# utra-robosoccer/Bez_IsaacGym

Measured on AMD Instinct MI355X. Metric: env-steps/s at num_envs=4096 (random-action rollout, bez_kick), higher is better.
Workload: dtype f32

## Files before the change

### bez_isaacgym_amd/csrc/bez_policy.hip

```cpp
#include <hip/hip_fp16.h>
#include <hip/hip_runtime.h>
#include <stdint.h>
#include <cstdlib>
#include <cstring>

#include <type_traits>

#include "../../include/bez_sim.h"
#include "bez_dr_noise.h"
#include "bez_dr_step.h"
#include "bez_ppo_loss.h"

namespace {

using half8 = __attribute__((ext_vector_type(8))) _Float16;
using f32x16 = __attribute__((ext_vector_type(16))) float;
using f32x2 = __attribute__((ext_vector_type(2))) float;
using half2v = __attribute__((ext_vector_type(2))) _Float16;
using half4v = __attribute__((ext_vector_type(4))) _Float16;

constexpr int PF_ROWS = 64;
constexpr int PF_MAXW = 416;
constexpr int PF_LD = PF_MAXW + 8;
constexpr int PF_MAXL = 6;
constexpr int PF_WAVES = 8;

struct PolicyArgs {
  const float* obs; int64_t n; int d_in;
  const double* mean; const double* var; float eps;
  int nhid;
  const _Float16* w[PF_MAXL]; const _Float16* b[PF_MAXL]; int width[PF_MAXL];
  const _Float16* w_mu; const _Float16* b_mu; int num_actions;
  const _Float16* w_val; const _Float16* b_val;
  float* mu; float* value;
  const float* logstd; const float* noise; const float* dones; const double* vmean; const double* vvar; float veps;
  float* mb_obs; float* mb_dones; float* mb_mu; float* mb_val; float* act; float* act_env; float* neglogp; float* sigma;
  BezPpoRolloutPost post;
  BezPpoActionNoise an;
  int dr_on; bez::dr::DrArgs dr;
  int64_t ld_obs, ld_act, ld_one;
  _Float16* x0_out; _Float16* act_out[PF_MAXL];
  int packed;
#ifdef BEZ_PF_STAMPS
  unsigned long long* stamps;
#endif
};
#ifdef BEZ_PF_STAMPS
#define PF_STAMP(k) do { if (a.stamps && blockIdx.x == 0 && threadIdx.x == 0) a.stamps[k] = __builtin_amdgcn_s_memtime(); } while (0)
__device__ unsigned long long* g_pf_wave_stamps = nullptr;
#define PF_WSTAMP(tag, wave, ph) do { if (g_pf_wave_stamps && blockIdx.x == 0 && (threadIdx.x & 63) == 0) g_pf_wave_stamps[(tag) * 64 + (wave) * 4 + (ph)] = __builtin_amdgcn_s_memtime(); } while (0)
#else
#define PF_STAMP(k) do { } while (0)
#define PF_WSTAMP(tag, wave, ph) do { } while (0)
#endif

template <int LD>
__device__ __forceinline__ void store_tile(const _Float16 (*src)[LD], _Float16* dst, int64_t row0, int nrow, int cols, int tid, int nw = PF_WAVES) {
  const int lane = tid & 63, wave = tid >> 6;
  if ((cols & 3) == 0) {
    const int c4 = cols >> 2;
    for (int rr = wave; rr < nrow; rr += nw) {
      _Float16* drow = dst + (row0 + rr) * cols;
      for (int c = lane; c < c4; c += 64) *reinterpret_cast<uint2*>(drow + 4 * c) = *reinterpret_cast<const uint2*>(&src[rr][4 * c]);
    }
  } else {
    const int c2 = cols >> 1;
    for (int rr = wave; rr < nrow; rr += nw) {
      _Float16* drow = dst + (row0 + rr) * cols;
      for (int c = lane; c < c2; c += 64) *reinterpret_cast<uint32_t*>(drow + 2 * c) = *reinterpret_cast<const uint32_t*>(&src[rr][2 * c]);
    }
  }
}

struct __attribute__((packed, aligned(4))) H8 { _Float16 v[8]; };

__device__ __forceinline__ half8 load_w8(const _Float16* row, int k0, int cols) {
  half8 f;
  if (k0 + 8 <= cols && (cols & 1) == 0) {
    const H8 t = *reinterpret_cast<const H8*>(row + k0);
#pragma unroll
    for (int j = 0; j < 8; ++j) f[j] = t.v[j];
  } else {
#pragma unroll
    for (int j = 0; j < 8; ++j) f[j] = (k0 + j < cols) ? row[k0 + j] : (_Float16)0.f;
  }
  return f;
}

template <int LD>
__device__ __forceinline__ void gemm_col_block(const _Float16 (*src)[LD], const _Float16* wrow, bool live, int in, int r, int h, f32x16& acc0, f32x16& acc1) {
  const int full = ((in & 1) == 0) ? (in >> 4) : 0;
  const int ksteps = (in + 15) >> 4;
  int ks = 0;
  auto group = [&](auto G) {
    constexpr int g = decltype(G)::value;
    half8 bf[g];
#pragma unroll
    for (int u = 0; u < g; ++u) {
      if (live) {
        const H8 t = *reinterpret_cast<const H8*>(wrow + (ks + u) * 16 + 8 * h);
#pragma unroll
        for (int j = 0; j < 8; ++j) bf[u][j] = t.v[j];
      } else {
#pragma unroll
        for (int j = 0; j < 8; ++j) bf[u][j] = (_Float16)0.f;
      }
    }
#pragma unroll
    for (int u = 0; u < g; ++u) {
      const int k0 = (ks + u) * 16 + 8 * h;
      const half8 a0 = *reinterpret_cast<const half8*>(&src[r][k0]);
      const half8 a1 = *reinterpret_cast<const half8*>(&src[32 + r][k0]);
      acc0 = __builtin_amdgcn_mfma_f32_32x32x16_f16(a0, bf[u], acc0, 0, 0, 0);
      acc1 = __builtin_amdgcn_mfma_f32_32x32x16_f16(a1, bf[u], acc1, 0, 0, 0);
    }
    ks += g;
  };
  while (ks + 12 <= full) group(std::integral_constant<int, 12>{});
  while (ks + 4 <= full) group(std::integral_constant<int, 4>{});
  while (ks + 1 <= full) group(std::integral_constant<int, 1>{});
  for (; ks < ksteps; ++ks) {
    const int k0 = ks * 16 + 8 * h;
    const half8 bf = load_w8(wrow, k0, live ? in : 0);
    const half8 a0 = *reinterpret_cast<const half8*>(&src[r][k0]);
    const half8 a1 = *reinterpret_cast<const half8*>(&src[32 + r][k0]);
    acc0 = __builtin_amdgcn_mfma_f32_32x32x16_f16(a0, bf, acc0, 0, 0, 0);
    acc1 = __builtin_amdgcn_mfma_f32_32x32x16_f16(a1, bf, acc1, 0, 0, 0);
  }
}

struct alignas(4) BiasQuad { half2v lo, hi; };
struct Bias16 { BiasQuad q[4]; };
__device__ __forceinline__ Bias16 load_bias16(const _Float16* B, int cb, int out) {
  Bias16 b;
  const half2v z = half2v{(_Float16)0.f, (_Float16)0.f};
  if (!B) {
#pragma unroll
    for (int j = 0; j < 4; ++j) { b.q[j].lo = z; b.q[j].hi = z; }
  } else if (((out & 3) | (int)(reinterpret_cast<uintptr_t>(B) & 3)) == 0) {
#pragma unroll
    for (int j = 0; j < 4; ++j) {
      const int c = cb + 8 * j;
      b.q[j] = *reinterpret_cast<const BiasQuad*>(B + (c < out ? c : 0));
    }
  } else {
#pragma unroll
    for (int j = 0; j < 4; ++j) {
      const int c = cb + 8 * j;
      b.q[j].lo = half2v{B[c < out ? c : 0], B[c + 1 < out ? c + 1 : 0]};
      b.q[j].hi = half2v{B[c + 2 < out ? c + 2 : 0], B[c + 3 < out ? c + 3 : 0]};
    }
  }
  return b;
}
constexpr int PF_G = 4;
template <int LD, bool T, int NACC, int RP>
__device__ __forceinline__ void gemm_packed(const _Float16 (*src)[LD], const _Float16* wblk, int ksteps, int r, int h, int half, f32x16* acc,
                                            const Bias16* bias = nullptr) {
  const _Float16* p = wblk + (h * 32 + r) * 8;
  auto fetch = [&](half8* f, int g) {
#pragma unroll
    for (int u = 0; u < PF_G; ++u) {
      const int k = g * PF_G + u < ksteps ? g * PF_G + u : ksteps - 1;
      f[u] = *reinterpret_cast<const half8*>(p + (size_t)k * 512);
    }
    __builtin_amdgcn_sched_barrier(0);
  };
  auto mma = [&](const half8& w, int ks) {
    const int k0 = ks * 16 + 8 * h;
    if (NACC == 2) {
      const half8 a0 = *reinterpret_cast<const half8*>(&src[r][k0]);
      const half8 a1 = *reinterpret_cast<const half8*>(&src[32 + r][k0]);
      acc[0] = T ? __builtin_amdgcn_mfma_f32_32x32x16_f16(w, a0, acc[0], 0, 0, 0) : __builtin_amdgcn_mfma_f32_32x32x16_f16(a0, w, acc[0], 0, 0, 0);
      acc[NACC - 1] = T ? __builtin_amdgcn_mfma_f32_32x32x16_f16(w, a1, acc[NACC - 1], 0, 0, 0) : __builtin_amdgcn_mfma_f32_32x32x16_f16(a1, w, acc[NACC - 1], 0, 0, 0);
    } else {
      const half8 a0 = *reinterpret_cast<const half8*>(&src[32 * half + r][k0]);
      acc[0] = T ? __builtin_amdgcn_mfma_f32_32x32x16_f16(w, a0, acc[0], 0, 0, 0) : __builtin_amdgcn_mfma_f32_32x32x16_f16(a0, w, acc[0], 0, 0, 0);
    }
  };
  auto stage = [&](const half8* f, int ks, auto CNT) {
#pragma unroll
    for (int u = 0; u < decltype(CNT)::value; ++u) mma(f[u], ks + u);
    __builtin_amdgcn_sched_barrier(0);
  };
  using Full = std::integral_constant<int, PF_G>;
  const int npair = ksteps / (2 * PF_G);
  half8 fa[PF_G], fb[PF_G];
  __builtin_amdgcn_sched_barrier(0);
  fetch(fa, 0);
#pragma unroll
  for (int j = 0; j < 4; ++j) {
    f32x2 lo = {0.f, 0.f}, hi = {0.f, 0.f};
    if (T && bias) { lo = __builtin_convertvector(bias->q[j].lo, f32x2); hi = __builtin_convertvector(bias->q[j].hi, f32x2); }
#pragma unroll
    for (int c = 0; c < NACC; ++c) { acc[c][4 * j] = lo.x; acc[c][4 * j + 1] = lo.y; acc[c][4 * j + 2] = hi.x; acc[c][4 * j + 3] = hi.y; }
  }
  __builtin_amdgcn_sched_barrier(0);
  for (int i = 0; i < npair; ++i) {
    fetch(fb, 2 * i + 1);
    stage(fa, 2 * i * PF_G, Full{});
    fetch(fa, 2 * i + 2);
    stage(fb, (2 * i + 1) * PF_G, Full{});
  }
  if constexpr (RP > PF_G) fetch(fb, 2 * npair + 1);
  if constexpr (RP > 0) stage(fa, 2 * npair * PF_G, std::integral_constant<int, (RP < PF_G ? RP : PF_G)>{});
  if constexpr (RP > PF_G) stage(fb, (2 * npair + 1) * PF_G, std::integral_constant<int, RP - PF_G>{});
}
template <class F>
__device__ __forceinline__ void dispatch_ksteps(int ksteps, F&& run) {
  static_assert(PF_G == 4, "eight remainders");
  switch (ksteps & 7) {
    case 0: run(std::integral_constant<int, 0>{}); break;
    case 1: run(std::integral_constant<int, 1>{}); break;
    case 2: run(std::integral_constant<int, 2>{}); break;
    case 3: run(std::integral_constant<int, 3>{}); break;
    case 4: run(std::integral_constant<int, 4>{}); break;
    case 5: run(std::integral_constant<int, 5>{}); break;
    case 6: run(std::integral_constant<int, 6>{}); break;
    default: run(std::integral_constant<int, 7>{}); break;
  }
}
template <bool ELU, int LDD>
__device__ __forceinline__ void store_row_groups(const f32x16& acc, _Float16 (*dst)[LDD], int row, int cb, int npad) {
#pragma unroll
  for (int j = 0; j < 4; ++j) {
    const int c0 = cb + 8 * j;
    uint32_t o[2];
#pragma unroll
    for (int q = 0; q < 2; ++q) {
      const int i = 4 * j + 2 * q;
      const half2v hq = __builtin_convertvector(f32x2{acc[i], acc[i + 1]}, half2v);
      if (ELU) {
        const f32x2 e = f32x2{__builtin_amdgcn_exp2f(__builtin_fmaf((float)hq.x, 1.4426950408889634f, 0.f)),
                              __builtin_amdgcn_exp2f(__builtin_fmaf((float)hq.y, 1.4426950408889634f, 0.f))} - f32x2{1.f, 1.f};
        const half2v eh = __builtin_convertvector(e, half2v);
        const uint32_t hb = __builtin_bit_cast(uint32_t, hq), eb = __builtin_bit_cast(uint32_t, eh);
        uint32_t neg;
        asm("v_pk_ashrrev_i16 %0, %1, %2" : "=v"(neg) : "v"(0x000f000fu), "v"(hb));
        o[q] = (eb & neg) | (hb & ~neg);
      } else {
        o[q] = __builtin_bit_cast(uint32_t, hq);
      }
    }
    if (LDD >= PF_LD || c0 < npad) *reinterpret_cast<uint2*>(&dst[row][c0]) = make_uint2(o[0], o[1]);
  }
}

template <bool ELU, bool PK, bool ONEHALF = false, int LDS, int LDD>
__device__ __forceinline__ void layer(const _Float16 (*src)[LDS], _Float16 (*dst)[LDD], const _Float16* W, const _Float16* B, int in, int out, int wave,
                                      int lane, int tag = 0, int nw = PF_WAVES) {
  const int r = lane & 31, h = lane >> 5;
  const int nblk = (out + 31) >> 5, npad = (out + 15) & ~15;
  if constexpr (PK && ONEHALF) {
    const int ksteps = (in + 15) >> 4;
    dispatch_ksteps(ksteps, [&](auto RP) {
      for (int nb = wave; nb < nblk; nb += nw) {
        const int cb = nb * 32 + 4 * h;
        const Bias16 bias = load_bias16(B, cb, out);
        f32x16 acc;
        if (nb == wave) PF_WSTAMP(tag, wave, 0);
        gemm_packed<LDS, true, 1, decltype(RP)::value>(src, W + (size_t)nb * ksteps * 512, ksteps, r, h, 0, &acc, &bias);
        if (nb == wave) PF_WSTAMP(tag, wave, 1);
        store_row_groups<ELU>(acc, dst, r, cb, npad);
        if (nb == wave) PF_WSTAMP(tag, wave, 2);
      }
    });
    return;
  }
  if constexpr (PK) {
    const int ksteps = (in + 15) >> 4;
    if (nblk * 2 <= PF_WAVES) {
      if (wave < 2 * nblk) {
        const int nb = wave < nblk ? wave : wave - nblk, half = wave < nblk ? 0 : 1, cb = nb * 32 + 4 * h;
        dispatch_ksteps(ksteps, [&](auto RP) {
          const Bias16 bias = load_bias16(B, cb, out);
          f32x16 acc;
          PF_WSTAMP(tag, wave, 0);
          gemm_packed<LDS, true, 1, decltype(RP)::value>(src, W + (size_t)nb * ksteps * 512, ksteps, r, h, half, &acc, &bias);
          PF_WSTAMP(tag, wave, 1);
          store_row_groups<ELU>(acc, dst, 32 * half + r, cb, npad);
          PF_WSTAMP(tag, wave, 2);
        });
      }
      return;
    }
    dispatch_ksteps(ksteps, [&](auto RP) {
      for (int nb = wave; nb < nblk; nb += nw) {
        const int cb = nb * 32 + 4 * h;
        const Bias16 bias = load_bias16(B, cb, out);
        f32x16 acc[2];
        if (nb == wave) PF_WSTAMP(tag, wave, 0);
        gemm_packed<LDS, true, 2, decltype(RP)::value>(src, W + (size_t)nb * ksteps * 512, ksteps, r, h, 0, acc, &bias);
        if (nb == wave) PF_WSTAMP(tag, wave, 1);
        store_row_groups<ELU>(acc[0], dst, r, cb, npad);
        store_row_groups<ELU>(acc[1], dst, 32 + r, cb, npad);
        if (nb == wave) PF_WSTAMP(tag, wave, 2); else PF_WSTAMP(tag, wave, 3);
      }
    });
    return;
  }
  for (int nb = wave; nb < nblk; nb += nw) {
    const int n = nb * 32 + r;
    const _Float16* wrow = W + (size_t)(n < out ? n : 0) * in;
    const float bias = (B && n < out) ? (float)B[n] : 0.f;
    f32x16 acc0, acc1;
#pragma unroll
    for (int i = 0; i < 16; ++i) { acc0[i] = bias; acc1[i] = bias; }
    gemm_col_block(src, wrow, n < out, in, r, h, acc0, acc1);
#pragma unroll
    for (int i = 0; i < 16; ++i) {
      const int row = (i & 3) + 8 * (i >> 2) + 4 * h;
      float v0 = (float)(_Float16)acc0[i], v1 = (float)(_Float16)acc1[i];
      if (ELU) { v0 = v0 > 0.f ? v0 : __expf(v0) - 1.f; v1 = v1 > 0.f ? v1 : __expf(v1) - 1.f; }
      if (LDD >= PF_LD || n < npad) {
        dst[row][n] = (_Float16)v0;
        dst[32 + row][n] = (_Float16)v1;
      }
    }
  }
}

template <bool ROLL, bool PK, int LD>
__device__ __forceinline__ void heads(const PolicyArgs& a, const _Float16 (*src)[LD], int in, float* tile, int64_t row0, int nrow, int lane) {
  const int r = lane & 31, h = lane >> 5, A = a.num_actions;
  const _Float16* wrow = r < A ? a.w_mu + (size_t)r * in : a.w_val;
  const bool live = r <= A;
  f32x16 acc0, acc1;
#pragma unroll
  for (int i = 0; i < 16; ++i) { acc0[i] = 0.f; acc1[i] = 0.f; }
  static_assert(!PK, "the fragment-major instantiations use heads_half");
  gemm_col_block(src, wrow, live, in, r, h, acc0, acc1);
  const float bias = r < A ? (float)a.b_mu[r] : (r == A ? (float)a.b_val[0] : 0.f);
#pragma unroll
  for (int i = 0; i < 16; ++i) {
    const int row = (i & 3) + 8 * (i >> 2) + 4 * h;
    const float v0 = (float)(_Float16)(acc0[i] + bias), v1 = (float)(_Float16)(acc1[i] + bias);
    if (ROLL) {
      if (r <= A) { tile[row * 33 + r] = v0; tile[(32 + row) * 33 + r] = v1; }
    } else {
      if (row < nrow) { if (r < A) a.mu[(row0 + row) * A + r] = v0; else if (r == A) a.value[row0 + row] = v0; }
      if (32 + row < nrow) { if (r < A) a.mu[(row0 + 32 + row) * A + r] = v1; else if (r == A) a.value[row0 + 32 + row] = v1; }
    }
  }
}

__device__ __forceinline__ float head_bias(const PolicyArgs& a, int r) {
  return r < a.num_actions ? (float)a.b_mu[r] : (r == a.num_actions ? (float)a.b_val[0] : 0.f);
}
template <bool ROLL, int LD>
__device__ __forceinline__ void heads_half(const PolicyArgs& a, const _Float16 (*src)[LD], int in, float* tile, int64_t row0, int nrow, int lane, int half) {
  const int r = lane & 31, h = lane >> 5, A = a.num_actions, ksteps = (in + 15) >> 4;
  const float bias = head_bias(a, r);
  dispatch_ksteps(ksteps, [&](auto RP) {
    f32x16 acc;
    gemm_packed<LD, false, 1, decltype(RP)::value>(src, a.w_mu, ksteps, r, h, half, &acc);
#pragma unroll
    for (int i = 0; i < 16; ++i) {
      const int row = 32 * half + (i & 3) + 8 * (i >> 2) + 4 * h;
      const float v = (float)(_Float16)(acc[i] + bias);
      if (ROLL) {
        if (r <= A) tile[row * 33 + r] = v;
      } else if (row < nrow) {
        if (r < A) a.mu[(row0 + row) * A + r] = v; else if (r == A) a.value[row0 + row] = v;
      }
    }
  });
}

constexpr int PF_FWD_WAVES = 16;
template <int MODE, int LD0, int LD1, bool PK, int ROWS = PF_ROWS>
__global__ __launch_bounds__(MODE == 2 ? PF_WAVES * 64 : PF_FWD_WAVES * 64, (MODE != 2 || (LD0 + LD1) * PF_ROWS * 2 <= 80 * 1024) ? 4 : 2) void policy_forward_kernel(PolicyArgs a) {
  constexpr bool ROLL = MODE == 1, TRAIN = MODE == 2;
  static_assert(ROWS == PF_ROWS || (ROWS == 32 && PK && MODE != 2), "32-row tiles: fragment-major weights, forward-only / rollout kernels");
  constexpr bool ONEHALF = ROWS == 32;
  __shared__ __attribute__((aligned(16))) _Float16 t0[ROWS][LD0];
  __shared__ __attribute__((aligned(16))) _Float16 t1[ROWS][LD1];
  const int tid = threadIdx.x, lane = tid & 63, wave = tid >> 6;
  constexpr int nw = MODE == 2 ? PF_WAVES : PF_FWD_WAVES, nt = nw * 64;
  if (ROLL && a.dr_on && blockIdx.x == gridDim.x - 1) {
    int* scratch = reinterpret_cast<int*>(&t0[0][0]);
    constexpr int cap = (int)(sizeof(t0) / sizeof(int)) - 1;
    bez::dr::dr_step(a.dr, scratch + 1, cap, scratch);
    return;
  }
  const int64_t row0 = (int64_t)blockIdx.x * ROWS;
  const int nrow = (int)((a.n - row0) < (int64_t)ROWS ? (a.n - row0) : (int64_t)ROWS);
  PF_STAMP(0);
  __shared__ float nzs[ROLL ? ROWS * 32 : 1];
  if (ROLL && a.an.snap_dev) {
    const bez::DrSnap sn = *static_cast<const bez::DrSnap*>(a.an.snap_dev);
    const unsigned long long frame = (unsigned long long)sn.frame_hi << 32 | sn.frame_lo;
    const int nel = nrow * a.num_actions;
    for (int q = tid; 4 * q < nel; q += nt) {
      float z4[4];
      bez::dr_noise_quad(a.an.seed, a.an.env_id_offset, frame, 1, ((row0 * a.num_actions) >> 2) + q, z4);
#pragma unroll
      for (int c = 0; c < 4; ++c) nzs[4 * q + c] = fmaf(z4[c], sn.sd, sn.mean);
    }
  }
  const int kpad0 = (a.d_in + 15) & ~15;
  for (int k = lane; k < kpad0; k += 64) {
    const bool kin = k < a.d_in;
    float mk = 0.f, sk = 1.f;
    if (a.mean && kin) { mk = (float)a.mean[k]; sk = sqrtf((float)a.var[k] + a.eps); }
#pragma unroll 4
    for (int rr = wave; rr < ROWS; rr += nw) {
      float v = 0.f;
      if (rr < nrow && kin) {
        v = a.obs[(row0 + rr) * a.d_in + k];
        if (ROLL) a.mb_obs[(row0 + rr) * a.ld_obs + k] = v;
        if (a.mean) {
          v = (v - mk) / sk;
          v = fminf(fmaxf(v, -5.0f), 5.0f);
        }
      }
      t0[rr][k] = (_Float16)v;
    }
  }
  __syncthreads();
  PF_STAMP(1);
  __shared__ float ls_s[1];
  [[maybe_unused]] double ep_c = 0.0, ep_r = 0.0, ep_l = 0.0;
  auto log_sigma_sum = [&]() {
    const int A = a.num_actions;
    const float lj = lane < A ? a.logstd[lane] : 0.f;
    float ls = 0.f;
    for (int j = 0; j < A; ++j) ls += __builtin_bit_cast(float, __builtin_amdgcn_readlane(__builtin_bit_cast(int, lj), j));
    if (lane == 0) ls_s[0] = ls;
  };
  auto bookkeeping = [&]() {
    const BezPpoRolloutPost& q = a.post;
    const bool ok = lane < nrow;
    const int64_t i = row0 + (ok ? lane : 0);
    double c = 0.0, r = 0.0, l = 0.0;
    if (ok) {
      const float rw = q.rew[i];
      float sh = rw * q.reward_scale;
      if (q.bootstrap) sh += q.gamma * q.prev_values[i] * (float)q.timeouts[i];
      q.shaped[i] = sh;
      const float d = (float)q.reset[i];
      q.dones_f[i] = d;
      a.mb_dones[i] = d;
      const float cr = q.cur_rew[i] + rw, cl = q.cur_len[i] + 1.0f;
      c = d; r = cr * d; l = cl * d;
      q.cur_rew[i] = cr * (1.0f - d); q.cur_len[i] = cl * (1.0f - d);
    }
    ep_c = c; ep_r = r; ep_l = l;
  };
  auto episode_sums = [&]() {
    double c = ep_c, r = ep_r, l = ep_l;
#pragma unroll
    for (int o = (ROWS < 64 ? ROWS : 64) / 2; o > 0; o >>= 1) { c += __shfl_xor(c, o, 64); r += __shfl_xor(r, o, 64); l += __shfl_xor(l, o, 64); }
    if (lane == 0 && c != 0.0) {
      if (a.post.ep_parts) {
        double* p = a.post.ep_parts + 4 * (size_t)blockIdx.x;
        p[0] += c; p[1] += r; p[2] += l;
      } else {
        atomicAdd(&a.post.ep_stats[0], c); atomicAdd(&a.post.ep_stats[1], r); atomicAdd(&a.post.ep_stats[2], l);
      }
    }
  };
  auto shadow_work = [&](int w) {
    if (!ROLL) return;
    if (w == 0 && wave == nw - 2) log_sigma_sum();
    if (a.post.rew && wave == nw - 1) {
      if (w == 0) bookkeeping();
      if (w == 1) episode_sums();
    }
  };
  shadow_work(0);
  if (TRAIN) store_tile(t0, a.x0_out, row0, nrow, a.d_in, tid, nw);
  int in = a.d_in;
  for (int L = 0; L < a.nhid; L += 2) {
    layer<true, PK, ONEHALF>(t0, t1, a.w[L], a.b[L], in, a.width[L], wave, lane, L, nw);
    PF_STAMP(2 + 2 * L);
    __syncthreads();
    PF_STAMP(3 + 2 * L);
    shadow_work(L + 1);
    in = a.width[L];
    if (TRAIN) store_tile(t1, a.act_out[L], row0, nrow, in, tid, nw);
    if (L + 1 < a.nhid) {
      layer<true, PK, ONEHALF>(t1, t0, a.w[L + 1], a.b[L + 1], in, a.width[L + 1], wave, lane, L + 1, nw);
      PF_STAMP(4 + 2 * L);
      __syncthreads();
      PF_STAMP(5 + 2 * L);
      in = a.width[L + 1];
      if (TRAIN) store_tile(t0, a.act_out[L + 1], row0, nrow, in, tid, nw);
    }
  }
  const bool in_t1 = (a.nhid & 1) != 0;
  float* tile = in_t1 ? reinterpret_cast<float*>(&t0[0][0]) : reinterpret_cast<float*>(&t1[0][0]);
  constexpr int NIT = ROLL ? (ROWS * 31 + nt - 1) / nt : 1;
  [[maybe_unused]] float ez[NIT], el[NIT];
  if (ROLL) {
    const int A = a.num_actions;
#pragma unroll
    for (int it = 0; it < NIT; ++it) {
      const int idx = tid + it * nt;
      ez[it] = el[it] = 0.f;
      if (idx < nrow * A) { ez[it] = a.noise[row0 * A + idx]; el[it] = a.logstd[idx % A]; }
    }
  }
  if constexpr (PK) {
    if (wave < (ONEHALF ? 1 : 2)) {
      if (in_t1) heads_half<ROLL>(a, t1, in, tile, row0, nrow, lane, wave);
      else heads_half<ROLL>(a, t0, in, tile, row0, nrow, lane, wave);
    }
  } else if (wave == 0) {
    if (in_t1) heads<ROLL, PK>(a, t1, in, tile, row0, nrow, lane);
    else heads<ROLL, PK>(a, t0, in, tile, row0, nrow, lane);
  }
  PF_STAMP(14);
  if (ROLL) {
    __syncthreads();
    const int A = a.num_actions;
    float* zz = tile + ROWS * 33;
    static_assert(sizeof(float) * ROWS * (33 + 36) <= sizeof(_Float16) * ROWS * (LD0 < LD1 ? LD0 : LD1), "the free tile holds both");
#pragma unroll
    for (int it = 0; it < NIT; ++it) {
      const int idx = tid + it * nt;
      if (idx >= nrow * A) break;
      const int rr = idx / A, j = idx - rr * A;
      const float m = tile[rr * 33 + j];
      const float l = el[it], sg = expf(l), z = ez[it];
      const float x = fmaf(sg, z, m);
      const int64_t o = (row0 + rr) * A + j;
      float xe = fminf(fmaxf(x, -1.0f), 1.0f);
      if (a.an.snap_dev) xe = xe + nzs[idx];
      const int64_t om = (row0 + rr) * a.ld_act + j;
      a.mb_mu[om] = m; a.act[om] = x; a.act_env[o] = xe; a.sigma[om] = sg;
      const float q = (x - m) / sg;
      zz[rr * 36 + j] = q * q;
    }
    __syncthreads();
    PF_STAMP(13);
    if (tid < nrow) {
      float acc = 0.f;
      const float4* z4 = reinterpret_cast<const float4*>(zz + tid * 36);
      for (int j = 0; j < A; j += 4) {
        const float4 v = z4[j >> 2];
        acc += v.x;
        if (j + 1 < A) acc += v.y;
        if (j + 2 < A) acc += v.z;
        if (j + 3 < A) acc += v.w;
      }
      a.neglogp[(row0 + tid) * a.ld_one] = 0.5f * acc + 0.5f * 1.8378770664093453f * (float)A + ls_s[0];
      float v = tile[tid * 33 + A];
      if (a.vmean) v = sqrtf((float)a.vvar[0] + a.veps) * fminf(fmaxf(v, -5.0f), 5.0f) + (float)a.vmean[0];
      a.mb_val[row0 + tid] = v;
      if (!a.post.rew) a.mb_dones[row0 + tid] = a.dones[row0 + tid];
    }
    PF_STAMP(12);
  }
  PF_STAMP(15);
}

struct BackwardArgs {
  int64_t n; int nhid; int width[PF_MAXL]; int num_actions;
  const float* gmu; const float* gval;
  const _Float16* act[PF_MAXL];
  const _Float16* wt[PF_MAXL];
  const _Float16* wht;
  _Float16* gz[PF_MAXL];
  _Float16* gmu16; _Float16* gv16;
  float* bgrad[PF_MAXL]; float* bmu_grad; float* bv_grad;
  int packed;
  float* partial; int ptotal; int poff[PF_MAXL];
  int prow;
  bez_loss::LossArgs loss;
};

template <int LA, int LB>
__device__ __forceinline__ void backward_elementwise_x4(const BackwardArgs& a, _Float16 (*A)[LA], _Float16 (*B)[LB], int L, int64_t row0, int tid, int wave,
                                                        int lane) {
  const int W = a.width[L], g = W >> 2;
  int P = 64, sh = 6;
  while (P > 1 && (P >> 1) >= g) { P >>= 1; --sh; }
  const int rp = 64 >> sh, lp = lane & (P - 1), sub = lane >> sh;
  const int npass = (g + 63) >> 6;
  float* red = reinterpret_cast<float*>(&B[0][0]);
  static_assert(sizeof(_Float16) * PF_ROWS * LB >= sizeof(float) * 8 * PF_MAXW, "the free tile holds the column-sum partials");
  const _Float16* act = a.act[L] + row0 * W;
  _Float16* gz = a.gz[L] + row0 * W;
  const int r0 = wave * rp + sub, rstep = PF_WAVES * rp, niter = PF_ROWS / rstep;
  for (int j = 0; j < npass; ++j) {
    const int cg = lp + 64 * j;
    f32x2 s01 = {0.f, 0.f}, s23 = {0.f, 0.f};
    if (cg < g) {
      constexpr int NB = 8;
      uint2 yy[NB], gg[NB];
#pragma unroll
      for (int i = 0; i < NB; ++i) {
        const int rr = r0 + i * rstep;
        if (i < niter) {
          yy[i] = *reinterpret_cast<const uint2*>(act + (size_t)rr * W + 4 * cg);
          gg[i] = *reinterpret_cast<const uint2*>(&A[rr][4 * cg]);
        }
      }
#pragma unroll
      for (int i = 0; i < NB; ++i) {
        const int rr = r0 + i * rstep;
        if (i < niter) {
          uint32_t zz[2];
#pragma unroll
          for (int q = 0; q < 2; ++q) {
            const half2v y = __builtin_bit_cast(half2v, q ? yy[i].y : yy[i].x), gq = __builtin_bit_cast(half2v, q ? gg[i].y : gg[i].x);
            const half2v yn = __builtin_elementwise_min(y, half2v{(_Float16)0.f, (_Float16)0.f});
            const half2v z = __builtin_convertvector(f32x2{__builtin_fmaf((float)gq.x, (float)yn.x, (float)gq.x), __builtin_fmaf((float)gq.y, (float)yn.y, (float)gq.y)}, half2v);
            zz[q] = __builtin_bit_cast(uint32_t, z);
            f32x2& sacc = q ? s23 : s01;
            sacc = f32x2{__builtin_fmaf((float)z.x, 1.f, sacc.x), __builtin_fmaf((float)z.y, 1.f, sacc.y)};
          }
          *reinterpret_cast<uint2*>(&A[rr][4 * cg]) = make_uint2(zz[0], zz[1]);
          *reinterpret_cast<uint2*>(gz + (size_t)rr * W + 4 * cg) = make_uint2(zz[0], zz[1]);
        }
      }
      *reinterpret_cast<float4*>(red + (size_t)r0 * W + 4 * cg) = make_float4(s01.x, s01.y, s23.x, s23.y);
    }
  }
  __syncthreads();
  if (tid < W) {
    float sum = 0.f;
    const int parts = PF_WAVES * rp;
    for (int q = 0; q < parts; ++q) sum += red[q * W + tid];
    a.partial[(size_t)blockIdx.x * a.prow + a.poff[L] + tid] = sum;
  }
}

template <bool PK, int LA, int LB>
__device__ __forceinline__ void backward_stage(const BackwardArgs& a, _Float16 (*A)[LA], _Float16 (*B)[LB], int L, int64_t row0, int nrow, int tid,
                                               int wave, int lane) {
  constexpr int NT = PF_WAVES * 64;
  const int W = a.width[L];
  if ((W & 3) == 0 && nrow == PF_ROWS) {
    backward_elementwise_x4(a, A, B, L, row0, tid, wave, lane);
  } else {
    float2* red = reinterpret_cast<float2*>(&B[0][0]);
    static_assert(sizeof(_Float16) * PF_ROWS * LB >= sizeof(float2) * NT, "the free tile holds the reduction scratch");
    const int ncp = W >> 1, nparts = NT / ncp;
    const int part = tid / ncp, cp = tid - part * ncp;
    float2 acc = make_float2(0.f, 0.f);
    if (part < nparts) {
      for (int rb = part; rb < nrow; rb += 8 * nparts) {
        uint32_t yy[8], gy[8];
#pragma unroll
        for (int u = 0; u < 8; ++u) {
          const int rr = rb + u * nparts;
          yy[u] = 0u; gy[u] = 0u;
          if (rr < nrow) {
            yy[u] = *reinterpret_cast<const uint32_t*>(a.act[L] + (row0 + rr) * W + 2 * cp);
            gy[u] = *reinterpret_cast<const uint32_t*>(&A[rr][2 * cp]);
          }
        }
#pragma unroll
        for (int u = 0; u < 8; ++u) {
          const int rr = rb + u * nparts;
          if (rr < nrow) {
            const _Float16 g0 = reinterpret_cast<const _Float16*>(&gy[u])[0], g1 = reinterpret_cast<const _Float16*>(&gy[u])[1];
            const float y0 = (float)reinterpret_cast<const _Float16*>(&yy[u])[0], y1 = (float)reinterpret_cast<const _Float16*>(&yy[u])[1];
            _Float16 z[2];
            z[0] = (_Float16)((float)g0 * (y0 > 0.f ? 1.f : y0 + 1.f));
            z[1] = (_Float16)((float)g1 * (y1 > 0.f ? 1.f : y1 + 1.f));
            const uint32_t zz = *reinterpret_cast<const uint32_t*>(z);
            *reinterpret_cast<uint32_t*>(&A[rr][2 * cp]) = zz;
            *reinterpret_cast<uint32_t*>(a.gz[L] + (row0 + rr) * W + 2 * cp) = zz;
            acc.x += (float)z[0]; acc.y += (float)z[1];
          }
        }
      }
    }
    red[tid] = acc;
    __syncthreads();
    if (tid < ncp) {
      float sx = 0.f, sy = 0.f;
      for (int q = 0; q < nparts; ++q) { sx += red[q * ncp + tid].x; sy += red[q * ncp + tid].y; }
      float* dst = a.partial + (size_t)blockIdx.x * a.prow + a.poff[L] + 2 * tid;
      dst[0] = sx; dst[1] = sy;
    }
  }
  if (L > 0) {
    __syncthreads();
    layer<false, PK>(A, B, a.wt[L], nullptr, W, a.width[L - 1], wave, lane);
    __syncthreads();
  }
}

template <int LD0, int LD1, bool PK, int LA = 0>
__global__ __launch_bounds__(PF_WAVES * 64, ((LD0 + LD1) * PF_ROWS * 2 <= 80 * 1024) ? 4 : 2) void policy_backward_kernel(BackwardArgs a) {
  __shared__ __attribute__((aligned(16))) _Float16 t0[PF_ROWS][LD0];
  __shared__ __attribute__((aligned(16))) _Float16 t1[PF_ROWS][LD1];
  constexpr int NT = PF_WAVES * 64;
  const int tid = threadIdx.x, lane = tid & 63, wave = tid >> 6;
  const int64_t row0 = (int64_t)blockIdx.x * PF_ROWS;
  const int nrow = (int)((a.n - row0) < (int64_t)PF_ROWS ? (a.n - row0) : (int64_t)PF_ROWS);
  const int A = a.num_actions;
  constexpr int LOSS_FLOATS = LA > 0 ? bez_loss::loss_lds_floats(LA > 0 ? LA : 1) : 0;
  static_assert(sizeof(float) * (LOSS_FLOATS + NT) <= sizeof(_Float16) * PF_ROWS * LD1, "tile 1 holds the loss tile and the head stage's scratch");
  static_assert(bez_loss::LOSS_TB == PF_ROWS, "the loss tile is the backward tile");
  float* ltile = reinterpret_cast<float*>(&t1[0][0]);
  if constexpr (LA > 0) bez_loss::ppo_loss_tile<LA, true>(a.loss, ltile, tid);
  {
    float* red = ltile + LOSS_FLOATS;
    const float* lgv = ltile + 4 * PF_ROWS * (LA + 1) + 3 * bez_loss::LOSS_CW * PF_ROWS;
    const int k = tid & 31, rsub = tid >> 5;
    float acc = 0.f;
#pragma unroll
    for (int j = 0; j < PF_ROWS / (NT / 32); ++j) {
      const int rr = rsub + j * (NT / 32);
      float v = 0.f;
      if (rr < nrow) {
        if constexpr (LA > 0) v = k < A ? ltile[rr * (LA + 1) + k] : (k == A ? lgv[rr] : 0.f);
        else v = k < A ? a.gmu[(row0 + rr) * A + k] : (k == A ? a.gval[row0 + rr] : 0.f);
      }
      const _Float16 hv = (_Float16)v;
      t0[rr][k] = hv;
      if (rr < nrow) {
        if (k < A) a.gmu16[(row0 + rr) * A + k] = hv; else if (k == A) a.gv16[row0 + rr] = hv;
        acc += (float)hv;
      }
    }
    red[tid] = acc;
    __syncthreads();
    if (tid <= A) {
      float sum = 0.f;
      for (int q = 0; q < NT / 32; ++q) sum += red[q * 32 + tid];
      a.partial[(size_t)blockIdx.x * a.prow + a.ptotal + tid] = sum;
    }
    __syncthreads();
  }
  layer<false, PK>(t0, t1, a.wht, nullptr, 32, a.width[a.nhid - 1], wave, lane);
  __syncthreads();
  bool in1 = true;
  for (int L = a.nhid - 1; L >= 0; --L) {
    if (in1) backward_stage<PK>(a, t1, t0, L, row0, nrow, tid, wave, lane);
    else backward_stage<PK>(a, t0, t1, L, row0, nrow, tid, wave, lane);
    in1 = !in1;
  }
}

__global__ __launch_bounds__(1024) void policy_bias_reduce_kernel(BackwardArgs a, int nwg) {
  __shared__ float sh[16][64];
  const int l = threadIdx.x & 63, rl = threadIdx.x >> 6;
  const int c = blockIdx.x * 64 + l;
  const int ncol = a.ptotal + a.num_actions + 1;
  float s = 0.f;
  if (c < ncol) {
#pragma unroll 8
    for (int w = rl; w < nwg; w += 16) s += a.partial[(size_t)w * a.prow + c];
  }
  sh[rl][l] = s;
  __syncthreads();
  if (rl == 0 && c < ncol) {
    float t = 0.f;
#pragma unroll
    for (int q = 0; q < 16; ++q) t += sh[q][l];
    if (c >= a.ptotal) {
      const int k = c - a.ptotal;
      if (k < a.num_actions) a.bmu_grad[k] += t; else a.bv_grad[0] += t;
    } else {
      int L = 0;
      while (L + 1 < a.nhid && c >= a.poff[L + 1]) ++L;
      a.bgrad[L][c - a.poff[L]] += t;
    }
  }
}

__global__ void scatter2_f16_kernel(const _Float16* __restrict__ src, const int32_t* __restrict__ ma, const int32_t* __restrict__ mb, int64_t n,
                                    _Float16* __restrict__ dst) {
  const int64_t i = (int64_t)blockIdx.x * blockDim.x + threadIdx.x;
  if (i < n) { const _Float16 v = src[i]; const int32_t a = ma[i], b = mb[i]; if (a >= 0) dst[a] = v; if (b >= 0) dst[b] = v; }
}

__global__ void scatter_f16_kernel(const _Float16* __restrict__ src, const int32_t* __restrict__ map, int64_t n, _Float16* __restrict__ dst) {
  const int64_t i = (int64_t)blockIdx.x * blockDim.x + threadIdx.x;
  if (i < n) { const int32_t m = map[i]; if (m >= 0) dst[m] = src[i]; }
}

}

#ifdef BEZ_PF_STAMPS
static unsigned long long* g_pf_stamps = nullptr;
extern "C" void bez_ppo_policy_debug_stamps(unsigned long long* dev) {
  g_pf_stamps = dev;
  unsigned long long* w = dev ? dev + 16 : nullptr;
  (void)hipMemcpyToSymbol(HIP_SYMBOL(g_pf_wave_stamps), &w, sizeof(w));
}
#endif
static int fill_args(PolicyArgs& a, const float* obs_dev, int64_t n, int32_t num_obs, const double* obs_mean_dev, const double* obs_var_dev, float obs_eps,
                     int32_t num_hidden, const void* const* hidden_w_f16_dev, const void* const* hidden_b_f16_dev, const int32_t* hidden_width,
                     const void* mu_w_f16_dev, const void* mu_b_f16_dev, int32_t num_actions, const void* value_w_f16_dev, const void* value_b_f16_dev) {
  if (!obs_dev || n <= 0 || num_obs <= 0 || num_obs > PF_MAXW || num_hidden <= 0 || num_hidden > PF_MAXL || !hidden_w_f16_dev || !hidden_b_f16_dev ||
      !hidden_width || !mu_w_f16_dev || !mu_b_f16_dev || !value_w_f16_dev || !value_b_f16_dev || num_actions <= 0 || num_actions > 31 ||
      (obs_mean_dev && !obs_var_dev)) return -1;
  a.obs = obs_dev; a.n = n; a.d_in = num_obs; a.mean = obs_mean_dev; a.var = obs_var_dev; a.eps = obs_eps; a.nhid = num_hidden;
  for (int i = 0; i < PF_MAXL; ++i) { a.w[i] = nullptr; a.b[i] = nullptr; a.width[i] = 0; }
  for (int i = 0; i < num_hidden; ++i) {
    if (!hidden_w_f16_dev[i] || !hidden_b_f16_dev[i] || hidden_width[i] <= 0 || hidden_width[i] > PF_MAXW) return -1;
    a.w[i] = (const _Float16*)hidden_w_f16_dev[i]; a.b[i] = (const _Float16*)hidden_b_f16_dev[i]; a.width[i] = hidden_width[i];
  }
  a.w_mu = (const _Float16*)mu_w_f16_dev; a.b_mu = (const _Float16*)mu_b_f16_dev; a.num_actions = num_actions;
  a.w_val = (const _Float16*)value_w_f16_dev; a.b_val = (const _Float16*)value_b_f16_dev;
  a.mu = nullptr; a.value = nullptr;
  a.logstd = a.noise = a.dones = nullptr; a.vmean = a.vvar = nullptr; a.veps = 0.f;
  a.mb_obs = a.mb_dones = a.mb_mu = a.mb_val = a.act = a.act_env = a.neglogp = a.sigma = nullptr;
  a.post = BezPpoRolloutPost{};
  a.an = BezPpoActionNoise{};
  a.dr_on = 0;
  a.ld_obs = num_obs; a.ld_act = num_actions; a.ld_one = 1;
  a.x0_out = nullptr;
  for (int i = 0; i < PF_MAXL; ++i) a.act_out[i] = nullptr;
  a.packed = 0;
#ifdef BEZ_PF_STAMPS
  a.stamps = g_pf_stamps;
#endif
  return 0;
}

static bool small_batch(int64_t n) {
  static const bool off = [] { const char* e = std::getenv("BEZ_PF_ROWS"); return e && std::atoi(e) == 64; }();
  return !off && n <= 8192;
}

extern "C" int bez_ppo_policy_forward(const float* obs_dev, int64_t n, int32_t num_obs, const double* obs_mean_dev, const double* obs_var_dev, float obs_eps,
                                      int32_t num_hidden, const void* const* hidden_w_f16_dev, const void* const* hidden_b_f16_dev, const int32_t* hidden_width,
                                      const void* mu_w_f16_dev, const void* mu_b_f16_dev, int32_t num_actions, const void* value_w_f16_dev,
                                      const void* value_b_f16_dev, float* mu_dev, float* value_dev, int32_t weights_packed, void* stream) {
  PolicyArgs a;
  if (!mu_dev || !value_dev || fill_args(a, obs_dev, n, num_obs, obs_mean_dev, obs_var_dev, obs_eps, num_hidden, hidden_w_f16_dev, hidden_b_f16_dev, hidden_width,
                                         mu_w_f16_dev, mu_b_f16_dev, num_actions, value_w_f16_dev, value_b_f16_dev)) return -1;
  a.mu = mu_dev; a.value = value_dev; a.packed = weights_packed;
  if (weights_packed && small_batch(n)) hipLaunchKernelGGL((policy_forward_kernel<0, PF_LD, PF_LD, true, 32>), dim3((unsigned)((n + 31) / 32)), dim3(PF_FWD_WAVES * 64), 0, (hipStream_t)stream, a);
  else if (weights_packed) hipLaunchKernelGGL((policy_forward_kernel<0, PF_LD, PF_LD, true>), dim3((unsigned)((n + PF_ROWS - 1) / PF_ROWS)), dim3(PF_FWD_WAVES * 64), 0, (hipStream_t)stream, a);
  else hipLaunchKernelGGL((policy_forward_kernel<0, PF_LD, PF_LD, false>), dim3((unsigned)((n + PF_ROWS - 1) / PF_ROWS)), dim3(PF_FWD_WAVES * 64), 0, (hipStream_t)stream, a);
  return hipGetLastError() == hipSuccess ? 0 : -2;
}

extern "C" int bez_ppo_policy_rollout_step(const float* obs_dev, int64_t n, int32_t num_obs, const double* obs_mean_dev, const double* obs_var_dev, float obs_eps,
                                           int32_t num_hidden, const void* const* hidden_w_f16_dev, const void* const* hidden_b_f16_dev,
                                           const int32_t* hidden_width, const void* mu_w_f16_dev, const void* mu_b_f16_dev, int32_t num_actions,
                                           const void* value_w_f16_dev, const void* value_b_f16_dev, const float* logstd_dev, const float* noise_dev,
                                           const float* dones_dev, const double* value_mean_dev, const double* value_var_dev, float value_eps, float* mb_obs_dev,
                                           float* mb_dones_dev, float* mb_mu_dev, float* mb_val_dev, float* actions_dev, float* env_actions_dev,
                                           float* neglogp_dev, float* sigma_dev, int32_t weights_packed, const BezPpoRolloutPost* prev_post, const BezPpoActionNoise* action_noise,
                                           const void* dr_step, const BezPpoRolloutLayout* layout, void* stream) {
  PolicyArgs a;
  if (prev_post && (!prev_post->rew || !prev_post->reset || !prev_post->timeouts || !prev_post->prev_values || !prev_post->shaped || !prev_post->dones_f ||
                    !prev_post->cur_rew || !prev_post->cur_len || !prev_post->ep_stats)) return -1;
  if (!logstd_dev || !noise_dev || !dones_dev || !mb_obs_dev || !mb_dones_dev || !mb_mu_dev || !mb_val_dev || !actions_dev || !env_actions_dev || !neglogp_dev ||
      !sigma_dev || (value_mean_dev && !value_var_dev) ||
      fill_args(a, obs_dev, n, num_obs, obs_mean_dev, obs_var_dev, obs_eps, num_hidden, hidden_w_f16_dev, hidden_b_f16_dev, hidden_width, mu_w_f16_dev,
                mu_b_f16_dev, num_actions, value_w_f16_dev, value_b_f16_dev)) return -1;
  a.logstd = logstd_dev; a.noise = noise_dev; a.dones = dones_dev; a.vmean = value_mean_dev; a.vvar = value_var_dev; a.veps = value_eps;
  a.mb_obs = mb_obs_dev; a.mb_dones = mb_dones_dev; a.mb_mu = mb_mu_dev; a.mb_val = mb_val_dev; a.act = actions_dev; a.act_env = env_actions_dev;
  a.neglogp = neglogp_dev; a.sigma = sigma_dev; a.packed = weights_packed;
  if (prev_post) a.post = *prev_post;
  if (action_noise && action_noise->snap_dev) a.an = *action_noise;
  if (layout) {
    if (layout->obs_row_stride < num_obs || layout->act_row_stride < num_actions || layout->scalar_stride < 1) return -1;
    a.ld_obs = layout->obs_row_stride; a.ld_act = layout->act_row_stride; a.ld_one = layout->scalar_stride;
  }
  static_assert(sizeof(bez::dr::DrArgs) <= BEZ_DR_STEP_BYTES, "BezPpoDrStep blob of the C ABI too small");
  if (dr_step) { std::memcpy(&a.dr, dr_step, sizeof(a.dr)); a.dr_on = 1; if (a.dr.n <= 0 || !a.dr.st || a.dr.first) return -1; }
  const bool small = weights_packed && small_batch(n);
  const int rows = small ? 32 : PF_ROWS;
  const unsigned grid = (unsigned)((n + rows - 1) / rows) + (dr_step ? 1u : 0u);
  if (small) hipLaunchKernelGGL((policy_forward_kernel<1, PF_LD, PF_LD, true, 32>), dim3(grid), dim3(PF_FWD_WAVES * 64), 0, (hipStream_t)stream, a);
  else if (weights_packed) hipLaunchKernelGGL((policy_forward_kernel<1, PF_LD, PF_LD, true>), dim3(grid), dim3(PF_FWD_WAVES * 64), 0, (hipStream_t)stream, a);
  else hipLaunchKernelGGL((policy_forward_kernel<1, PF_LD, PF_LD, false>), dim3(grid), dim3(PF_FWD_WAVES * 64), 0, (hipStream_t)stream, a);
  return hipGetLastError() == hipSuccess ? 0 : -2;
}

extern "C" int bez_ppo_policy_forward_train(const float* obs_dev, int64_t n, int32_t num_obs, const double* obs_mean_dev, const double* obs_var_dev, float obs_eps,
                                            int32_t num_hidden, const void* const* hidden_w_f16_dev, const void* const* hidden_b_f16_dev,
                                            const int32_t* hidden_width, const void* mu_w_f16_dev, const void* mu_b_f16_dev, int32_t num_actions,
                                            const void* value_w_f16_dev, const void* value_b_f16_dev, void* x0_f16_dev, void* const* act_f16_dev,
                                            float* mu_dev, float* value_dev, int32_t weights_packed, void* stream) {
  PolicyArgs a;
  if (!mu_dev || !value_dev || !x0_f16_dev || !act_f16_dev || (num_obs & 1) ||
      fill_args(a, obs_dev, n, num_obs, obs_mean_dev, obs_var_dev, obs_eps, num_hidden, hidden_w_f16_dev, hidden_b_f16_dev, hidden_width, mu_w_f16_dev,
                mu_b_f16_dev, num_actions, value_w_f16_dev, value_b_f16_dev)) return -1;
  for (int i = 0; i < num_hidden; ++i) {
    if (!act_f16_dev[i] || (hidden_width[i] & 1)) return -1;
    a.act_out[i] = (_Float16*)act_f16_dev[i];
  }
  a.x0_out = (_Float16*)x0_f16_dev; a.mu = mu_dev; a.value = value_dev; a.packed = weights_packed;
  int w0 = num_obs, w1 = 0;
  for (int i = 0; i < num_hidden; ++i) { int& w = (i & 1) ? w0 : w1; if (hidden_width[i] > w) w = hidden_width[i]; }
  const dim3 grid((unsigned)((n + PF_ROWS - 1) / PF_ROWS)), block(PF_WAVES * 64);
// ... 88 lines not shown
```

Baseline: 148.1 million.

## Prefetch next layer's first weight group and bias across layer boundaries

Adds a cross-layer lookahead so that each wave issues global loads for the first weight k-group (and bias) of its next block or next layer before the barrier and epilogue of the current one. The forward pass (one-half mode) chains through the hidden layers into the heads, and the backward pass chains through the transposed layers. The aim is to hide weight-load latency at each layer start behind the store and sync of the previous layer. The cost is extra live registers and more template complexity, which may lower occupancy. Wave index is also made uniform via readfirstlane.

```diff
diff --git a/bez_isaacgym_amd/csrc/bez_policy.hip b/bez_isaacgym_amd/csrc/bez_policy.hip
--- a/bez_isaacgym_amd/csrc/bez_policy.hip
+++ b/bez_isaacgym_amd/csrc/bez_policy.hip
@@ -154,18 +154,58 @@
   return b;
 }
 constexpr int PF_G = 4;
-template <int LD, bool T, int NACC, int RP>
+__device__ __forceinline__ void fetch_group(half8* f, const _Float16* p, int g, int ksteps) {
+#pragma unroll
+  for (int u = 0; u < PF_G; ++u) {
+    const int k = g * PF_G + u < ksteps ? g * PF_G + u : ksteps - 1;
+    f[u] = *reinterpret_cast<const half8*>(p + (size_t)k * 512);
+  }
+  __builtin_amdgcn_sched_barrier(0);
+}
+struct Ahead { half8 fa[PF_G]; Bias16 bias; };
+__device__ __forceinline__ void forget_bias(Ahead& ah) {
+#pragma unroll
+  for (int j = 0; j < 4; ++j) { ah.bias.q[j].lo = __builtin_nondeterministic_value(ah.bias.q[j].lo); ah.bias.q[j].hi = __builtin_nondeterministic_value(ah.bias.q[j].hi); }
+}
+__device__ __forceinline__ void forget(Ahead& ah) {
+#pragma unroll
+  for (int u = 0; u < PF_G; ++u) ah.fa[u] = __builtin_nondeterministic_value(ah.fa[u]);
+  forget_bias(ah);
+}
+template <bool BIAS>
+__device__ __forceinline__ void request_block(Ahead& ah, const _Float16* W, const _Float16* B, int nb, int ksteps, int out, int lane) {
+  const int r = lane & 31, h = lane >> 5;
+  __builtin_amdgcn_sched_barrier(0);
+  int cb = nb * 32 + 4 * h, lo = (h * 32 + r) * 8;
+  asm volatile("" : "+v"(cb), "+v"(lo));
+  __builtin_assume(!BIAS || B != nullptr);
+  if (BIAS) ah.bias = load_bias16(B, cb, out); else forget_bias(ah);
+  fetch_group(ah.fa, W + (size_t)nb * ksteps * 512 + lo, 0, ksteps);
+}
+struct Unit { int nb, half; bool any; };
+template <bool ONEHALF>
+__device__ __forceinline__ Unit first_unit(int out, int wave) {
+  const int nblk = (out + 31) >> 5;
+  if (!ONEHALF && nblk * 2 <= PF_WAVES) return Unit{wave < nblk ? wave : wave - nblk, wave < nblk ? 0 : 1, wave < 2 * nblk};
+  return Unit{wave, 0, wave < nblk};
+}
+template <bool ONEHALF, bool BIAS>
+__device__ __forceinline__ void request_unit(Ahead& ah, const _Float16* W, const _Float16* B, int in, int out, int wave, int lane) {
+  const Unit u = first_unit<ONEHALF>(out, wave);
+  if (u.any) request_block<BIAS>(ah, W, B, u.nb, (in + 15) >> 4, out, lane); else forget(ah);
+}
+struct NoNext { __device__ __forceinline__ void operator()() const {} };
+#ifndef BEZ_PF_AHEAD_FORWARD
+#define BEZ_PF_AHEAD_FORWARD 1
+#endif
+#ifndef BEZ_PF_AHEAD_BACKWARD
+#define BEZ_PF_AHEAD_BACKWARD 1
+#endif
+template <int LD, bool T, int NACC, int RP, bool PRE = false>
 __device__ __forceinline__ void gemm_packed(const _Float16 (*src)[LD], const _Float16* wblk, int ksteps, int r, int h, int half, f32x16* acc,
-                                            const Bias16* bias = nullptr) {
+                                            const Bias16* bias = nullptr, half8* pre = nullptr) {
   const _Float16* p = wblk + (h * 32 + r) * 8;
-  auto fetch = [&](half8* f, int g) {
-#pragma unroll
-    for (int u = 0; u < PF_G; ++u) {
-      const int k = g * PF_G + u < ksteps ? g * PF_G + u : ksteps - 1;
-      f[u] = *reinterpret_cast<const half8*>(p + (size_t)k * 512);
-    }
-    __builtin_amdgcn_sched_barrier(0);
-  };
+  auto fetch = [&](half8* f, int g) { fetch_group(f, p, g, ksteps); };
   auto mma = [&](const half8& w, int ks) {
     const int k0 = ks * 16 + 8 * h;
     if (NACC == 2) {
@@ -185,9 +225,10 @@
   };
   using Full = std::integral_constant<int, PF_G>;
   const int npair = ksteps / (2 * PF_G);
-  half8 fa[PF_G], fb[PF_G];
+  half8 own[PF_G], fb[PF_G];
+  half8* fa = PRE ? pre : own;
   __builtin_amdgcn_sched_barrier(0);
-  fetch(fa, 0);
+  if constexpr (!PRE) fetch(fa, 0);
 #pragma unroll
   for (int j = 0; j < 4; ++j) {
     f32x2 lo = {0.f, 0.f}, hi = {0.f, 0.f};
@@ -246,11 +287,70 @@
   }
 }
 
-template <bool ELU, bool PK, bool ONEHALF = false, int LDS, int LDD>
+template <bool ELU, bool PK, bool ONEHALF = false, bool AHEAD = false, int LDS, int LDD, class NEXT = NoNext>
 __device__ __forceinline__ void layer(const _Float16 (*src)[LDS], _Float16 (*dst)[LDD], const _Float16* W, const _Float16* B, int in, int out, int wave,
-                                      int lane, int tag = 0, int nw = PF_WAVES) {
-  const int r = lane & 31, h = lane >> 5;
+                                      int lane, int tag = 0, int nw = PF_WAVES,
+                                      Ahead* ahp = nullptr, NEXT next = NEXT{}) {
+  int r = lane & 31, h = lane >> 5;
+  if constexpr (PK && AHEAD) asm volatile("" : "+v"(r), "+v"(h));
   const int nblk = (out + 31) >> 5, npad = (out + 15) & ~15;
+  if constexpr (PK && AHEAD) {
+    constexpr bool BIAS = ELU;
+    Ahead& ah = *ahp;
+    const int ksteps = (in + 15) >> 4;
+    const Bias16* bias = BIAS ? &ah.bias : nullptr;
+    if (!first_unit<ONEHALF>(out, wave).any) {
+      next();
+      return;
+    }
+    auto request_behind = [&](int nb2) __attribute__((always_inline)) {
+      if (nb2 < nblk) request_block<BIAS>(ah, W, B, nb2, ksteps, out, lane);
+      else next();
+    };
+    if constexpr (ONEHALF) {
+      dispatch_ksteps(ksteps, [&](auto RP) {
+        for (int nb = wave; nb < nblk; nb += nw) {
+          const int cb = nb * 32 + 4 * h;
+          f32x16 acc;
+          if (nb == wave) PF_WSTAMP(tag, wave, 0);
+          gemm_packed<LDS, true, 1, decltype(RP)::value, true>(src, W + (size_t)nb * ksteps * 512, ksteps, r, h, 0, &acc, bias, ah.fa);
+          request_behind(nb + nw);
+          if (nb == wave) PF_WSTAMP(tag, wave, 1);
+          store_row_groups<ELU>(acc, dst, r, cb, npad);
+          if (nb == wave) PF_WSTAMP(tag, wave, 2);
+        }
+      });
+      return;
+    }
+    if (nblk * 2 <= PF_WAVES) {
+      const Unit u = first_unit<false>(out, wave);
+      const int nb = u.nb, half = u.half, cb = nb * 32 + 4 * h;
+      dispatch_ksteps(ksteps, [&](auto RP) {
+        f32x16 acc;
+        PF_WSTAMP(tag, wave, 0);
+        gemm_packed<LDS, true, 1, decltype(RP)::value, true>(src, W + (size_t)nb * ksteps * 512, ksteps, r, h, half, &acc, bias, ah.fa);
+        request_behind(nblk);
+        PF_WSTAMP(tag, wave, 1);
+        store_row_groups<ELU>(acc, dst, 32 * half + r, cb, npad);
+        PF_WSTAMP(tag, wave, 2);
+      });
+      return;
+    }
+    dispatch_ksteps(ksteps, [&](auto RP) {
+      for (int nb = wave; nb < nblk; nb += nw) {
+        const int cb = nb * 32 + 4 * h;
+        f32x16 acc[2];
+        if (nb == wave) PF_WSTAMP(tag, wave, 0);
+        gemm_packed<LDS, true, 2, decltype(RP)::value, true>(src, W + (size_t)nb * ksteps * 512, ksteps, r, h, 0, acc, bias, ah.fa);
+        request_behind(nb + nw);
+        if (nb == wave) PF_WSTAMP(tag, wave, 1);
+        store_row_groups<ELU>(acc[0], dst, r, cb, npad);
+        store_row_groups<ELU>(acc[1], dst, 32 + r, cb, npad);
+        if (nb == wave) PF_WSTAMP(tag, wave, 2); else PF_WSTAMP(tag, wave, 3);
+      }
+    });
+    return;
+  }
   if constexpr (PK && ONEHALF) {
     const int ksteps = (in + 15) >> 4;
     dispatch_ksteps(ksteps, [&](auto RP) {
@@ -347,13 +447,14 @@
 __device__ __forceinline__ float head_bias(const PolicyArgs& a, int r) {
   return r < a.num_actions ? (float)a.b_mu[r] : (r == a.num_actions ? (float)a.b_val[0] : 0.f);
 }
-template <bool ROLL, int LD>
-__device__ __forceinline__ void heads_half(const PolicyArgs& a, const _Float16 (*src)[LD], int in, float* tile, int64_t row0, int nrow, int lane, int half) {
+template <bool ROLL, bool AHEAD, int LD>
+__device__ __forceinline__ void heads_half(const PolicyArgs& a, const _Float16 (*src)[LD], int in, float* tile, int64_t row0, int nrow, int lane, int half,
+                                           half8* pre, float pre_bias) {
   const int r = lane & 31, h = lane >> 5, A = a.num_actions, ksteps = (in + 15) >> 4;
-  const float bias = head_bias(a, r);
+  const float bias = AHEAD ? pre_bias : head_bias(a, r);
   dispatch_ksteps(ksteps, [&](auto RP) {
     f32x16 acc;
-    gemm_packed<LD, false, 1, decltype(RP)::value>(src, a.w_mu, ksteps, r, h, half, &acc);
+    gemm_packed<LD, false, 1, decltype(RP)::value, AHEAD>(src, a.w_mu, ksteps, r, h, half, &acc, nullptr, pre);
 #pragma unroll
     for (int i = 0; i < 16; ++i) {
       const int row = 32 * half + (i & 3) + 8 * (i >> 2) + 4 * h;
@@ -375,7 +476,7 @@
   constexpr bool ONEHALF = ROWS == 32;
   __shared__ __attribute__((aligned(16))) _Float16 t0[ROWS][LD0];
   __shared__ __attribute__((aligned(16))) _Float16 t1[ROWS][LD1];
-  const int tid = threadIdx.x, lane = tid & 63, wave = tid >> 6;
+  const int tid = threadIdx.x, lane = tid & 63, wave = __builtin_amdgcn_readfirstlane(tid >> 6);
   constexpr int nw = MODE == 2 ? PF_WAVES : PF_FWD_WAVES, nt = nw * 64;
   if (ROLL && a.dr_on && blockIdx.x == gridDim.x - 1) {
     int* scratch = reinterpret_cast<int*>(&t0[0][0]);
@@ -386,6 +487,23 @@
   const int64_t row0 = (int64_t)blockIdx.x * ROWS;
   const int nrow = (int)((a.n - row0) < (int64_t)ROWS ? (a.n - row0) : (int64_t)ROWS);
   PF_STAMP(0);
+  constexpr bool AHEAD = PK && ONEHALF && BEZ_PF_AHEAD_FORWARD != 0;
+  [[maybe_unused]] Ahead ah;
+  [[maybe_unused]] float hbias = 0.f;
+  struct Product { const _Float16* W; const _Float16* B; int in, out; bool heads; };
+  [[maybe_unused]] auto product = [&](int P) {
+    if (P < a.nhid) return Product{a.w[P], a.b[P], P ? a.width[P - 1] : a.d_in, a.width[P], false};
+    return Product{a.w_mu, nullptr, a.width[a.nhid - 1], a.num_actions + 1, true};
+  };
+  [[maybe_unused]] auto request_product = [&](const Product& q) __attribute__((always_inline)) {
+    if (!q.heads) {
+      request_unit<ONEHALF, true>(ah, q.W, q.B, q.in, q.out, wave, lane);
+    } else if (wave < (ONEHALF ? 1 : 2)) {
+      hbias = head_bias(a, lane & 31);
+      request_unit<ONEHALF, false>(ah, q.W, nullptr, q.in, q.out, wave, lane);
+    }
+  };
+  if constexpr (AHEAD) request_product(product(0));
   __shared__ float nzs[ROLL ? ROWS * 32 : 1];
   if (ROLL && a.an.snap_dev) {
     const bez::DrSnap sn = *static_cast<const bez::DrSnap*>(a.an.snap_dev);
@@ -472,7 +590,8 @@
   if (TRAIN) store_tile(t0, a.x0_out, row0, nrow, a.d_in, tid, nw);
   int in = a.d_in;
   for (int L = 0; L < a.nhid; L += 2) {
-    layer<true, PK, ONEHALF>(t0, t1, a.w[L], a.b[L], in, a.width[L], wave, lane, L, nw);
+    [[maybe_unused]] Product nx = AHEAD ? product(L + 1) : Product{};
+    layer<true, PK, ONEHALF, AHEAD>(t0, t1, a.w[L], a.b[L], in, a.width[L], wave, lane, L, nw, &ah, [&]() __attribute__((always_inline)) { request_product(nx); });
     PF_STAMP(2 + 2 * L);
     __syncthreads();
     PF_STAMP(3 + 2 * L);
@@ -480,7 +599,8 @@
     in = a.width[L];
     if (TRAIN) store_tile(t1, a.act_out[L], row0, nrow, in, tid, nw);
     if (L + 1 < a.nhid) {
-      layer<true, PK, ONEHALF>(t1, t0, a.w[L + 1], a.b[L + 1], in, a.width[L + 1], wave, lane, L + 1, nw);
+      if constexpr (AHEAD) nx = product(L + 2);
+      layer<true, PK, ONEHALF, AHEAD>(t1, t0, a.w[L + 1], a.b[L + 1], in, a.width[L + 1], wave, lane, L + 1, nw, &ah, [&]() __attribute__((always_inline)) { request_product(nx); });
       PF_STAMP(4 + 2 * L);
       __syncthreads();
       PF_STAMP(5 + 2 * L);
@@ -503,8 +623,8 @@
   }
   if constexpr (PK) {
     if (wave < (ONEHALF ? 1 : 2)) {
-      if (in_t1) heads_half<ROLL>(a, t1, in, tile, row0, nrow, lane, wave);
-      else heads_half<ROLL>(a, t0, in, tile, row0, nrow, lane, wave);
+      if (in_t1) heads_half<ROLL, AHEAD>(a, t1, in, tile, row0, nrow, lane, wave, ah.fa, hbias);
+      else heads_half<ROLL, AHEAD>(a, t0, in, tile, row0, nrow, lane, wave, ah.fa, hbias);
     }
   } else if (wave == 0) {
     if (in_t1) heads<ROLL, PK>(a, t1, in, tile, row0, nrow, lane);
@@ -627,9 +747,9 @@
   }
 }
 
-template <bool PK, int LA, int LB>
+template <bool PK, bool AHEAD, int LA, int LB>
 __device__ __forceinline__ void backward_stage(const BackwardArgs& a, _Float16 (*A)[LA], _Float16 (*B)[LB], int L, int64_t row0, int nrow, int tid,
-                                               int wave, int lane) {
+                                               int wave, int lane, Ahead& ah) {
   constexpr int NT = PF_WAVES * 64;
   const int W = a.width[L];
   if ((W & 3) == 0 && nrow == PF_ROWS) {
@@ -680,7 +800,11 @@
   }
   if (L > 0) {
     __syncthreads();
-    layer<false, PK>(A, B, a.wt[L], nullptr, W, a.width[L - 1], wave, lane);
+    const _Float16* wn = L > 1 ? a.wt[L - 1] : nullptr;
+    const int inn = a.width[L - 1], outn = L > 1 ? a.width[L - 2] : 0;
+    layer<false, PK, false, AHEAD>(A, B, a.wt[L], nullptr, W, inn, wave, lane, 0, PF_WAVES, &ah, [&]() __attribute__((always_inline)) {
+      if (wn) request_unit<false, false>(ah, wn, nullptr, inn, outn, wave, lane);
+    });
     __syncthreads();
   }
 }
@@ -690,10 +814,13 @@
   __shared__ __attribute__((aligned(16))) _Float16 t0[PF_ROWS][LD0];
   __shared__ __attribute__((aligned(16))) _Float16 t1[PF_ROWS][LD1];
   constexpr int NT = PF_WAVES * 64;
-  const int tid = threadIdx.x, lane = tid & 63, wave = tid >> 6;
+  const int tid = threadIdx.x, lane = tid & 63, wave = __builtin_amdgcn_readfirstlane(tid >> 6);
   const int64_t row0 = (int64_t)blockIdx.x * PF_ROWS;
   const int nrow = (int)((a.n - row0) < (int64_t)PF_ROWS ? (a.n - row0) : (int64_t)PF_ROWS);
   const int A = a.num_actions;
+  constexpr bool AHEAD = PK && BEZ_PF_AHEAD_BACKWARD != 0;
+  [[maybe_unused]] Ahead ah;
+  if constexpr (AHEAD) request_unit<false, false>(ah, a.wht, nullptr, 32, a.width[a.nhid - 1], wave, lane);
   constexpr int LOSS_FLOATS = LA > 0 ? bez_loss::loss_lds_floats(LA > 0 ? LA : 1) : 0;
   static_assert(sizeof(float) * (LOSS_FLOATS + NT) <= sizeof(_Float16) * PF_ROWS * LD1, "tile 1 holds the loss tile and the head stage's scratch");
   static_assert(bez_loss::LOSS_TB == PF_ROWS, "the loss tile is the backward tile");
@@ -728,12 +855,16 @@
     }
     __syncthreads();
   }
-  layer<false, PK>(t0, t1, a.wht, nullptr, 32, a.width[a.nhid - 1], wave, lane);
+  const _Float16* wn = a.nhid > 1 ? a.wt[a.nhid - 1] : nullptr;
+  const int inn = a.width[a.nhid - 1], outn = a.nhid > 1 ? a.width[a.nhid - 2] : 0;
+  layer<false, PK, false, AHEAD>(t0, t1, a.wht, nullptr, 32, inn, wave, lane, 0, PF_WAVES, &ah, [&]() __attribute__((always_inline)) {
+    if (wn) request_unit<false, false>(ah, wn, nullptr, inn, outn, wave, lane);
+  });
   __syncthreads();
   bool in1 = true;
   for (int L = a.nhid - 1; L >= 0; --L) {
-    if (in1) backward_stage<PK>(a, t1, t0, L, row0, nrow, tid, wave, lane);
-    else backward_stage<PK>(a, t0, t1, L, row0, nrow, tid, wave, lane);
+    if (in1) backward_stage<PK, AHEAD>(a, t1, t0, L, row0, nrow, tid, wave, lane, ah);
+    else backward_stage<PK, AHEAD>(a, t0, t1, L, row0, nrow, tid, wave, lane, ah);
     in1 = !in1;
   }
 }
```

New measurement: 147.7 million, median of 2. Within noise of the previous version (-0.3%).
